# dylkot/cNMF

Hardware: AMD Instinct MI355X
Metric: NMF restarts/sec (50000x2000xK5..13) (higher is better)
Workload: dtype f32 (exact integer f16 plane x 2 f16 planes with per-row exponent, f32 accumulate)

## Files before the change

cnmf_amd/csrc/batch_host.hip.h:

```cpp
#pragma once

#include "batch_sched.h"

static_assert(PLAN_BK == BK && PLAN_G3_MW == G3_MW && PLAN_G3_JW == G3_JW && PLAN_G3C_JW == G3C_JW && PLAN_G3_BK == G3_BK &&
              PLAN_KSMALL == KSMALL, "pass_plan.h repeats the tile constants of the kernel headers");
static PadShape pad_shape(const cnmf_ctx* ctx) { return PadShape{ctx->N_pad, ctx->G_pad}; }
static int sweep_chunks(const cnmf_ctx* ctx, int L) { return sweep_chunks(ctx->knobs.sweep_parts, L); }
static int sweep_parts(const cnmf_ctx* ctx, int L) { return sweep_parts(ctx->knobs.sweep_parts, L); }

static int ensure_batch(cnmf_ctx* ctx, int KC, int max_k = KMAX, int min_k = 1)
{
    const bool use3 = gemm3_enabled(ctx, KC);
    const SplitCaps caps = size_splits(pad_shape(ctx), KC, use3, gemm3_wg_slots(ctx->knobs));
    const int nsplit = caps.nsplit, nsplitA = caps.nsplitA;
    const int parts = std::max(sweep_parts(ctx, (int)ctx->N), sweep_parts(ctx, (int)ctx->G));
    const size_t gp_need = (size_t)(KC / std::max(1, min_k) + 1) * parts * max_k * max_k;
    if (ctx->bat.kc == KC && ctx->bat.nsplit == nsplit && ctx->bat.nsplitA == nsplitA &&
        ctx->bat.parts == parts && ctx->bat.gram_part_floats >= gp_need && (!use3 || ctx->bat.H3)) return CNMF_OK;
    ctx->bat.release();
    OwnedLocal<BatchBuffersF> b;
    const size_t hb = (size_t)KC * ctx->G_pad * sizeof(float);
    const size_t wb = (size_t)KC * ctx->N_pad * sizeof(float);
    HIP_TRY(ctx, hipMalloc(&b.H, hb));
    HIP_TRY(ctx, hipMalloc(&b.Wt, wb));
// ... 62 lines not shown
        clk::time_point t0;
        bool timing = false;
        while (*flag != stamp) {
            if (++spins % 4096 != 0) continue;
            if (!timing) { t0 = clk::now(); timing = true; continue; }
            if (std::chrono::duration_cast<std::chrono::milliseconds>(clk::now() - t0).count() < 20) continue;
            t0 = clk::now();
            const hipError_t q = hipStreamQuery(ctx->stream);
            if (q == hipSuccess) {
                if (*flag == stamp) break;
                SET_ERR(ctx, "slot snapshot %d was never published (slot %d)", stamp, s);
                return CNMF_EHIP;
            }
            if (q != hipErrorNotReady) {
                SET_ERR(ctx, "stream failed while waiting for a slot snapshot: %s", hipGetErrorString(q));
                return CNMF_EHIP;
            }
        }
    }
    __atomic_thread_fence(__ATOMIC_ACQUIRE);
    return CNMF_OK;
}

static int validate_params(cnmf_ctx* ctx, const cnmf_cd_params* p)
{
    if (!p) { SET_ERR(ctx, "params is NULL"); return CNMF_EINVAL; }
    if (!(p->tol >= 0) || p->max_iter < 1) { SET_ERR(ctx, "bad tol/max_iter"); return CNMF_EINVAL; }
    if (p->l1_reg_W < 0 || p->l2_reg_W < 0 || p->l1_reg_H < 0 || p->l2_reg_H < 0) {
        SET_ERR(ctx, "negative regularisation"); return CNMF_EINVAL;
    }
    return CNMF_OK;
}

static_assert(SCHED_KMAX == KMAX && SCHED_RING == RING, "batch_sched.h repeats KMAX and RING");

struct PassScheme {
    bool use3 = false;
    bool usec = false;
    bool use2g = false;
    bool use2h = false;
    int mode = 0;
    XOperand xA{}, xB{};
    const double* dsc = nullptr;
    int jwA = G3_JW;
    int nsubA = 1, nsubB = 1, KbA = 0, KbB = 0;
    void leave_matrix_pipe() { use3 = usec = use2h = use2g = false; }
};

static int pick_scheme(cnmf_ctx* ctx, int KC, PassScheme* out)
{
    const CdKnobs& kn = ctx->knobs;
    PassScheme p;
    int rc;
    p.use3 = gemm3_enabled(ctx, KC);
    if (p.use3 && kn.gemm3 >= 3) {
        if ((rc = ensure_counts(ctx))) return rc;
        p.usec = ctx->counts.state == 1;
    }
    p.use2g = p.use3 && !p.usec && kn.gemm3 >= 4 && ctx->G_pad % G3C_JW == 0 && ctx->N_pad % G3C_JW == 0;
    if (p.use2g && (rc = ensure_x2planes(ctx))) return rc;
    p.use2h = (p.usec && ctx->counts.fmt == 4) || p.use2g;
    p.mode = !p.use3 ? 0 : (p.use2g ? 5 : (p.usec ? (p.use2h ? 4 : 3) : std::min(kn.gemm3, 2)));
    p.KbA = ctx->G_pad / 16; p.KbB = ctx->N_pad / 16;
    p.xA = p.use2g ? ctx->x2.passA() : ctx->counts.passA();
    p.xB = p.use2g ? ctx->x2.passB() : ctx->counts.passB();
    p.dsc = p.use2g ? nullptr : ctx->counts.d_scale;
    p.nsubA = p.use2h ? gemm2h_nsub(p.xA.hi != nullptr, p.KbA, kn.g2_nsub) : 1;
    p.nsubB = p.use2h ? gemm2h_nsub(p.xB.hi != nullptr, p.KbB, kn.g2_nsub) : 1;
    if (p.use3 && !p.usec && !p.use2g && (rc = ensure_planes(ctx))) return rc;
    p.jwA = (p.usec || p.use2g) ? G3C_JW : G3_JW;
    *out = p;
    return CNMF_OK;
}

struct BatchRun {
    cnmf_ctx* ctx; const cnmf_cd_params* prm; hipStream_t st;
    int n; const int32_t* kk; int init_mode; const double* avg; const float *W0, *H0;
    int32_t* n_iter_out; double* viol_out; bool resident;
    int N, G, max_k; int64_t total_k;
    std::vector<size_t> hoff, woff;
    DevPool pool;
    EventPool events;
    struct PinnedInts { int* p = nullptr; ~PinnedInts() { if (p) hipHostFree(p); } } repack_host;
    float *d_Hres = nullptr, *d_Wres = nullptr;
    float *d_H0 = nullptr, *d_Wt0 = nullptr;
    int* d_repack = nullptr;
    int n_repack = 0;
    PassScheme ps;
    bool fuseW = false;
    int shgen = 0;
    int* shW[2] = {nullptr, nullptr};
    bool h3_valid = false;
    int fin_y = 1, lag = 2;
    int chunksW, partsW, chunksH, partsH;
    float l1W, l2W, l1H, l2H;
    PassPlan plan;
    int time_stride = 0;
    std::vector<hipEvent_t> gev;
    hipEvent_t ev_begin = nullptr, ev_end = nullptr, ev_tail = nullptr;
    int nsplit3_first = 1;
    BatchSched sched;
    BatchRun(int n_, const int32_t* kk_, int KC, const double* hint, bool dbg) : n(n_), kk(kk_), sched(n_, kk_, KC, hint, dbg) {}
};

static int plan_passes(BatchRun& b, int cap, int capA)
{
    cnmf_ctx* ctx = b.ctx;
    PassPlan& p = b.plan;
    plan_pass_splits(p, pad_shape(ctx), b.sched.KC, b.ps.use3, b.ps.jwA, b.ps.nsubA, gemm3_wg_slots(ctx->knobs), ctx->knobs.no_streamk, cap, capA);
    const std::vector<unsigned char>* flags = b.ps.use3 ? (p.sk3.on ? &p.sk3.flags : nullptr) : (p.sk.on ? &p.sk.split : nullptr);
    if (flags) HIP_TRY(ctx, hipMemcpyAsync(ctx->bat.d_split, flags->data(), flags->size(), hipMemcpyHostToDevice, b.st));
    return CNMF_OK;
}

static int retire_slot(BatchRun& b, int s, const SlotDesc& snap)
{
    cnmf_ctx* ctx = b.ctx;
    hipStream_t st = b.st;
    const HostSlot& h = b.sched.hs[s];
    const int r = h.restart, k = h.k, N = b.N, G = b.G;
    dim3 gH((G + 255) / 256, k), gW((N + 255) / 256, k);
    extract_kernel<<<gH, 256, 0, st>>>(ctx->bat.H, ctx->G_pad, G, h.off, k, b.d_Hres + b.hoff[r], 0);
    if (b.d_Wres) extract_kernel<<<gW, 256, 0, st>>>(ctx->bat.Wt, ctx->N_pad, N, h.off, k, b.d_Wres + b.woff[r], 1);
    clear_rows_kernel<<<gH, 256, 0, st>>>(ctx->bat.H, ctx->G_pad, ctx->G_pad, h.off, k);
    clear_rows_kernel<<<gW, 256, 0, st>>>(ctx->bat.Wt, ctx->N_pad, ctx->N_pad, h.off, k);
    HIP_TRY(ctx, hipGetLastError());
    if (b.n_iter_out) b.n_iter_out[r] = snap.iter;
    if (b.viol_out) b.viol_out[r] = snap.viol_last;
    b.sched.retire(s, snap.iter);
    return CNMF_OK;
}

static int repack(BatchRun& b, int width, bool balanced = false)
{
    cnmf_ctx* ctx = b.ctx;
    hipStream_t st = b.st;
    const int KC0 = b.sched.KC0;
    int* hm = b.repack_host.p + (size_t)(b.n_repack++ % RING) * 3 * KC0;
    int* d_colmap = b.d_repack, *d_ids = b.d_repack + KC0, *d_offs = b.d_repack + 2 * KC0;
    const RepackPlan pl = b.sched.plan_repack(width, balanced, hm);
    if (pl.nmove || pl.pos < width) {
        HIP_TRY(ctx, hipMemcpyAsync(d_colmap, hm, (size_t)width * sizeof(int), hipMemcpyHostToDevice, st));
        gather_rows_cm_kernel<<<dim3((ctx->N_pad / 4 + 255) / 256, width), 256, 0, st>>>(ctx->bat.Wt, ctx->N_pad, d_colmap, ctx->bat.XHt);
        gather_rows_cm_kernel<<<dim3((ctx->G_pad / 4 + 255) / 256, width), 256, 0, st>>>(ctx->bat.H, ctx->G_pad, d_colmap, ctx->bat.XtW);
        HIP_TRY(ctx, hipGetLastError());
        HIP_TRY(ctx, hipMemcpyAsync(ctx->bat.Wt, ctx->bat.XHt, (size_t)width * ctx->N_pad * sizeof(float), hipMemcpyDeviceToDevice, st));
        HIP_TRY(ctx, hipMemcpyAsync(ctx->bat.H, ctx->bat.XtW, (size_t)width * ctx->G_pad * sizeof(float), hipMemcpyDeviceToDevice, st));
        if (b.fuseW) {
            int* tmp = ctx->bat.shiftW + 2 * ctx->bat.kc;
            for (int g2 = 0; g2 < 2; ++g2) {
                permute_ints_kernel<<<(width + 255) / 256, 256, 0, st>>>(b.shW[g2], d_colmap, tmp, width);
                HIP_TRY(ctx, hipMemcpyAsync(b.shW[g2], tmp, (size_t)width * sizeof(int), hipMemcpyDeviceToDevice, st));
            }
            HIP_TRY(ctx, hipGetLastError());
        }
        if (pl.nmove) {
            HIP_TRY(ctx, hipMemcpyAsync(d_ids, hm + KC0, (size_t)pl.nmove * sizeof(int), hipMemcpyHostToDevice, st));
            HIP_TRY(ctx, hipMemcpyAsync(d_offs, hm + 2 * KC0, (size_t)pl.nmove * sizeof(int), hipMemcpyHostToDevice, st));
            set_slot_offs_kernel<<<(pl.nmove + 255) / 256, 256, 0, st>>>(ctx->bat.d_slots, d_ids, d_offs, pl.nmove);
            HIP_TRY(ctx, hipGetLastError());
        }
    }
    b.h3_valid = false;
    if (b.ps.use2h) HIP_TRY(ctx, launch_rowmax_part(st, ctx->bat.Wt, ctx->N_pad, b.N, b.sched.KC, b.chunksW * 256, nullptr, b.partsW, ctx->bat.rmaxW));
    return CNMF_OK;
}

static int install(BatchRun& b, const Placement& p)
{
    cnmf_ctx* ctx = b.ctx;
    hipStream_t st = b.st;
    const int r = p.restart, k = p.k, off = p.off, N = b.N, G = b.G;
    dim3 gI((std::max(N, G) + 255) / 256, k);
    if (b.init_mode == 0) {
        HIP_TRY(ctx, hipMemcpyAsync(ctx->stageH, b.H0 + b.hoff[r], (size_t)k * G * sizeof(float), hipMemcpyHostToDevice, st));
        HIP_TRY(ctx, hipMemcpyAsync(ctx->stageW, b.W0 + b.woff[r], (size_t)k * N * sizeof(float), hipMemcpyHostToDevice, st));
        install_kernel<<<gI, 256, 0, st>>>(ctx->stageH, ctx->stageW, ctx->bat.H, ctx->G_pad, G, ctx->bat.Wt, ctx->N_pad, N, off, k);
    } else {
        install_cm_kernel<<<gI, 256, 0, st>>>(b.d_H0 + b.hoff[r], b.d_Wt0 + b.woff[r], ctx->bat.H, ctx->G_pad, G, ctx->bat.Wt, ctx->N_pad, N, off);
    }
    HIP_TRY(ctx, hipGetLastError());
    if (b.fuseW) {
        float mx = 0.f;
        if (b.init_mode == 1) mx = 6.0f * (float)b.avg[r];
        else for (size_t q = 0; q < (size_t)k * N; ++q) mx = std::max(mx, b.W0[b.woff[r] + q]);
        int e2 = 0;
        if (mx > 0.f) std::frexp(mx, &e2);
        const int sh0 = mx > 0.f ? std::max(-110, std::min(120, 13 - e2)) : 0;
        set_ints_kernel<<<1, 128, 0, st>>>(b.shW[0], b.shW[1], off, k, sh0);
        HIP_TRY(ctx, hipGetLastError());
    }
    SlotDesc* d = &ctx->bat.h_slots[p.slot];
    memset(d, 0, sizeof *d);
    d->off = off; d->k = k; d->active = 1; d->iter = 0; d->restart = r;
    HIP_TRY(ctx, hipMemcpyAsync(ctx->bat.d_slots + p.slot, d, sizeof(SlotDesc), hipMemcpyHostToDevice, st));
    return CNMF_OK;
}

static int refill(BatchRun& b, int& n_new)
{
    cnmf_ctx* ctx = b.ctx;
    BatchSched& sc = b.sched;
    n_new = 0;
    int* new_list = ctx->bat.h_slot_list + (size_t)(sc.it % RING) * sc.KC0;
    int rc;
    sc.begin_refill();
    while (true) {
        Placement p;
        while (sc.next_placement(&p)) {
            if ((rc = install(b, p))) return rc;
            new_list[n_new++] = p.slot;
        }
        if (!sc.defrag_due()) break;
        if ((rc = repack(b, sc.KC))) return rc;
        sc.defragmented();
    }
    if (n_new) {
        int* dl = ctx->bat.d_slot_list + (size_t)(sc.it % RING) * sc.KC0;
        HIP_TRY(ctx, hipMemcpyAsync(dl, new_list, n_new * sizeof(int), hipMemcpyHostToDevice, b.st));
        gram_rows_kernel<<<n_new, 256, 0, b.st>>>(ctx->bat.H, ctx->G_pad, b.G, ctx->bat.d_slots, dl, ctx->bat.gramH, b.l2W);
        HIP_TRY(ctx, hipGetLastError());
    }
    return CNMF_OK;
}

static int launch_pass_a(BatchRun& b, int n_new, unsigned long long livemask, hipEvent_t ev_begin, CutPlanes* cutA)
{
    cnmf_ctx* ctx = b.ctx;
    hipStream_t st = b.st;
    const PassScheme& ps = b.ps;
    const PassPlan& pl = b.plan;
    const int KC = b.sched.KC, gm = ctx->knobs.gemm3;
    const long long plane = (long long)KC * ctx->N_pad;
    *cutA = NO_CUT;
    if (!ps.use3) {
        if (pl.sk.on) {
            HIP_TRY(ctx, launch_streamk_passA(st, pl.sk, ctx->bat.H, ctx->G_pad, ctx->X, ctx->G_pad, ctx->bat.XHt,
                                              ctx->bat.XHt1, ctx->N_pad, ctx->N_pad));
            *cutA = CutPlanes{ctx->bat.XHt1, ctx->bat.d_split, 128, pl.sk.mw, pl.sk.MG, nullptr};
        } else
            HIP_TRY(ctx, launch_gemm<false>(st, 0, ctx->bat.H, ctx->G_pad, ctx->X, ctx->G_pad, ctx->bat.XHt,
                                            ctx->N_pad, plane, KC, ctx->G_pad, ctx->N_pad, pl.nsplitA));
        return CNMF_OK;
    }
    if ((n_new > 0 || !b.h3_valid) && ps.use2h) {
        HIP_TRY(ctx, launch_rowmax_part(st, ctx->bat.H, ctx->G_pad, b.G, KC, b.chunksH * 256, ps.dsc, b.partsH, ctx->bat.rmaxH));
        HIP_TRY(ctx, launch_split2h(st, ctx->bat.H, ctx->G_pad, KC, ctx->G_pad, ctx->bat.H3, G3_MW, ps.dsc, ctx->bat.rmaxH,
                                    b.partsH, ctx->bat.iscaleH));
    } else if (n_new > 0 || !b.h3_valid)
        HIP_TRY(ctx, launch_split3(st, ctx->bat.H, ctx->G_pad, KC, ctx->G_pad, ctx->bat.H3, G3_MW, ps.usec ? ctx->counts.d_scale : nullptr));
    if (ev_begin) hipEventRecord(ev_begin, st);
    if (ps.use2h) {
        G2Launch g;
        g.A2 = ctx->bat.H3; g.rscale = ctx->bat.iscaleH; g.x = ps.xA; g.Kb = ps.KbA;
        g.C[0] = ctx->bat.XHt; g.C[1] = ctx->bat.XHt1; g.C[2] = ctx->bat.XHt2; g.ldc = ctx->N_pad;
        g.livemask = livemask; g.kn = &ctx->knobs;
        if (pl.sk3.on) { g.sk = &pl.sk3; HIP_TRY(ctx, launch_gemm2h_streamk(st, g)); }
        else { g.cstride = plane; g.KC = KC; g.Jpad = ctx->N_pad; g.nsplit = pl.nsplitA; HIP_TRY(ctx, launch_gemm2h(st, g)); }
    } else if (pl.sk3.on) {
        if (ps.usec)
            HIP_TRY(ctx, launch_gemm3c_streamk(st, pl.sk3, ctx->bat.H3, ps.xA.plane, ps.xA.hi, ps.xA.flags, ctx->bat.XHt, ctx->bat.XHt1,
                                               ctx->bat.XHt2, ctx->N_pad));
        else
            HIP_TRY(ctx, launch_gemm3_streamk(st, pl.sk3, ctx->bat.H3, ctx->planes.X3, ctx->bat.XHt, ctx->bat.XHt1, ctx->bat.XHt2, ctx->N_pad, gm));
    } else if (ps.usec)
        HIP_TRY(ctx, launch_gemm3c(st, ctx->bat.H3, ps.xA.plane, ps.xA.hi, ps.xA.flags, ctx->G_pad / 16, ctx->bat.XHt, ctx->N_pad,
                                   plane, KC, ctx->N_pad, pl.nsplitA));
    else
        HIP_TRY(ctx, launch_gemm3(st, ctx->bat.H3, ctx->planes.X3, ctx->G_pad / 16, ctx->bat.XHt, ctx->N_pad,
                                  plane, KC, ctx->N_pad, pl.nsplitA, gm));
    if (pl.sk3.on) *cutA = CutPlanes{ctx->bat.XHt1, ctx->bat.d_split, ps.jwA, G3_MW, pl.sk3.MG, ctx->bat.XHt2};
    return CNMF_OK;
}

static void launch_finalize(BatchRun& b, const FinalizeArgs& fa)
{
    finalize_kernel<<<dim3(b.sched.nslots, b.fin_y), 256, 0, b.st>>>(fa.gram_part, fa.viol_part, fa.nparts, fa.gram_out, fa.l2_reg,
                                                                   fa.slots, fa.phase, fa.tol, fa.max_iter, fa.want_gram, fa.gld,
                                                                   fa.snap_out, fa.stamp);
}

static int launch_w_finalize(BatchRun& b)
{
    cnmf_ctx* ctx = b.ctx;
    const int KC = b.sched.KC, nslots = b.sched.nslots;
    const FinalizeArgs fa{ctx->bat.gram_part, ctx->bat.viol_part, b.partsW, ctx->bat.gramW, b.l2H, ctx->bat.d_slots, 0, b.prm->tol,
                          b.prm->max_iter, 1, b.max_k, nullptr, 0};
    if (b.ps.use2h) {
        const bool fuse_now = b.fuseW;
// ... 59 lines not shown
        HIP_TRY(ctx, launch_reduce_splits(b.st, ctx->bat.XtW, nsB, plane, plane, ps.usec ? ps.dsc : nullptr, ctx->G_pad));
    HIP_TRY(ctx, launch_sweep(b.st, s));
    return CNMF_OK;
}

static int launch_h_finalize(BatchRun& b)
{
    cnmf_ctx* ctx = b.ctx;
    const PassScheme& ps = b.ps;
    const BatchSched& sc = b.sched;
    SlotDesc* snap = ctx->bat.h_snap + (size_t)(sc.it % RING) * sc.KC0;
    SlotDesc* snap_dev = nullptr;
    HIP_TRY(ctx, hipHostGetDevicePointer((void**)&snap_dev, snap, 0));
    const FinalizeArgs fa{ctx->bat.gram_part, ctx->bat.viol_part, b.partsH, ctx->bat.gramH, b.l2W, ctx->bat.d_slots, 1, b.prm->tol,
                          b.prm->max_iter, 1, b.max_k, snap_dev, (int)(sc.it + 1)};
    if (ps.use2h)
        HIP_TRY(ctx, launch_split2h_finalize(b.st, ctx->bat.H, ctx->G_pad, sc.KC, ctx->G_pad, ctx->bat.H3, G3_MW, ps.dsc,
                                             ctx->bat.rmaxH, b.partsH, ctx->bat.iscaleH, fa, sc.nslots, b.fin_y));
    else if (ps.use3)
        HIP_TRY(ctx, launch_split3_finalize(b.st, ctx->bat.H, ctx->G_pad, sc.KC, ctx->G_pad, ctx->bat.H3, G3_MW,
                                            ps.usec ? ctx->counts.d_scale : nullptr, fa, sc.nslots, b.fin_y));
    else
        launch_finalize(b, fa);
    if (ps.use3) b.h3_valid = true;
    HIP_TRY(ctx, hipGetLastError());
    return CNMF_OK;
}

static int iterate(BatchRun& b, int n_new)
{
    cnmf_ctx* ctx = b.ctx;
    hipStream_t st = b.st;
    const PassScheme& ps = b.ps;
    BatchSched& sc = b.sched;
    int tiers = 0, rc;
    for (int s2 = 0; s2 < sc.nslots; ++s2)
        if (sc.hs[s2].state) tiers |= sc.hs[s2].k <= 16 ? 1 : (sc.hs[s2].k <= 32 ? 2 : (sc.hs[s2].k <= KSMALL ? 4 : 8));
    unsigned long long livemask = ~0ull;
    if (ps.use2h && sc.n_pending == 0 && ctx->knobs.part) {
        int fullest = 0;
        livemask = sc.live_tiles(&fullest);
        if (fullest > 6) livemask = ~0ull;
    }
    hipEvent_t* ev = nullptr;
    if (b.time_stride > 0 && sc.it % b.time_stride == 0) {
        for (int i = 0; i < 4; ++i) b.gev.push_back(b.events.get());
        POOL_TRY(ctx, b.events);
        ev = &b.gev[b.gev.size() - 4];
        hipEventRecord(ev[0], st);
    }
    SweepLaunch w = batch_sweep(ctx, sc.nslots, b.max_k, tiers);
    if ((rc = launch_pass_a(b, n_new, livemask, ev ? ev[0] : nullptr, &w.cut))) return rc;
    if (ev) hipEventRecord(ev[1], st);
    if (w.cut.plane1) w.from = SweepLaunch::CUT_PLANES;
    else
        HIP_TRY(ctx, launch_reduce_splits(st, ctx->bat.XHt, ps.use2h ? gemm2h_splits(ps.KbA, b.plan.nsplitA, ps.nsubA) : b.plan.nsplitA,
                                          (long long)sc.KC * ctx->N_pad, (long long)sc.KC * ctx->N_pad));
    w.V = ctx->bat.Wt; w.ldv = ctx->N_pad; w.L = b.N; w.P = ctx->bat.XHt; w.gram = ctx->bat.gramH; w.l1 = b.l1W;
    w.chunks = b.chunksW; w.parts = b.partsW; w.want_gram = 1;
    if (ps.use2h) w.rmax_part = ctx->bat.rmaxW;
    const PlaneOut wplanes{(unsigned short*)ctx->bat.Wt3, b.shW[b.shgen], ps.KbB, G3_MW};
    if (b.fuseW && ps.use2h) w.planes = &wplanes;
    HIP_TRY(ctx, launch_sweep(st, w));
    if ((rc = launch_w_finalize(b))) return rc;
    if (ev) hipEventRecord(ev[2], st);
    int nsB = 1;
    if ((rc = launch_pass_b(b, livemask, &nsB))) return rc;
    if (ev) hipEventRecord(ev[3], st);
    if ((rc = launch_h_sweep(b, tiers, nsB))) return rc;
    if ((rc = launch_h_finalize(b))) return rc;
    sc.end_iteration();
    return CNMF_OK;
}

static int inspect(BatchRun& b)
{
    BatchSched& sc = b.sched;
    const int64_t si = sc.it - 1 - b.lag;
    if (si < 0) return CNMF_OK;
    const SlotDesc* sp = b.ctx->bat.h_snap + (size_t)(si % RING) * sc.KC0;
    const int ns = sc.snap_nslots[si % RING];
    int rc = wait_snapshot(b.ctx, sp, ns, (int)(si + 1));
    if (rc) return rc;
    for (int s = 0; s < ns; ++s)
        if (sc.retirable(s, si, sp[s].active, sp[s].restart) && (rc = retire_slot(b, s, sp[s]))) return rc;
    sc.resort_pending();
    return CNMF_OK;
}

static int compact(BatchRun& b)
{
    BatchSched& sc = b.sched;
    PassScheme& ps = b.ps;
    if (!sc.in_tail()) return CNMF_OK;
    const bool part = b.ctx->knobs.part;
    const TailPlan t = sc.tail_plan(ps.use3, ps.usec, ps.use2h, part);
    int rc;
    if (t.rebalance) {
        if ((rc = repack(b, sc.KC, true))) return rc;
        sc.rebalanced();
    }
    if (t.width < sc.KC) {
        const int KC0 = sc.KC0;
        if ((rc = repack(b, t.width, t.stay3 && ps.use2h && part))) return rc;
        sc.narrowed(t.width);
        if (!t.stay3) ps.leave_matrix_pipe();
        if ((rc = plan_passes(b, (b.ctx->bat.nsplit * KC0) / sc.KC, (b.ctx->bat.nsplitA * KC0) / sc.KC))) return rc;
    }
    return CNMF_OK;
}

static int alloc_call_buffers(BatchRun& b, bool want_W)
{
    cnmf_ctx* ctx = b.ctx;
    const int G = b.G, n = b.n, KC0 = b.sched.KC0;
    if (b.resident) {
        if (ctx->spectra_rows && ctx->spectra_G != G) {
            SET_ERR(ctx, "the resident store holds spectra over %lld genes, this matrix has %d: cnmf_spectra_reset first",
                    (long long)ctx->spectra_G, G);
            return CNMF_ESTATE;
        }
        ctx->spectra_G = G;
        const size_t need = (ctx->spectra_rows + (size_t)b.total_k) * G;
        if (need > ctx->spectra_cap) {
            float* nb = nullptr;
            const size_t cap = std::max(need, ctx->spectra_cap * 2);
            HIP_TRY(ctx, hipMalloc(&nb, cap * sizeof(float)));
            hipError_t ce = hipSuccess;
            if (ctx->spectra_rows)
                ce = hipMemcpyAsync(nb, ctx->spectra, ctx->spectra_rows * G * sizeof(float), hipMemcpyDeviceToDevice, b.st);
            if (ce == hipSuccess) ce = hipStreamSynchronize(b.st);
            if (ce != hipSuccess) { hipFree(nb); HIP_TRY(ctx, ce); }
            hipFree(ctx->spectra);
            ctx->spectra = nb; ctx->spectra_cap = cap;
        }
        b.d_Hres = ctx->spectra + ctx->spectra_rows * G;
    } else {
        b.d_Hres = b.pool.get<float>(b.hoff[n]);
    }
    if (want_W) b.d_Wres = b.pool.get<float>(b.woff[n]);
    b.d_repack = b.pool.get<int>((size_t)3 * KC0);
    POOL_TRY(ctx, b.pool);
    HIP_TRY(ctx, hipHostMalloc(&b.repack_host.p, (size_t)RING * 3 * KC0 * sizeof(int)));
    return CNMF_OK;
}

static int generate_inits(BatchRun& b, const uint32_t* seeds)
{
    cnmf_ctx* ctx = b.ctx;
    const int n = b.n, N = b.N, G = b.G;
    b.d_H0 = b.pool.get<float>(b.hoff[n]);
    b.d_Wt0 = b.pool.get<float>(b.woff[n]);
    RngJob* d_jobs = b.pool.get<RngJob>((size_t)n);
    POOL_TRY(ctx, b.pool);
    std::vector<RngJob> jobs(n);
    int rowoff = 0;
    for (int r = 0; r < n; ++r) {
        jobs[r] = RngJob{seeds[r], b.kk[r], rowoff, b.avg[r], (long long)b.kk[r] * ((long long)G + N)};
        rowoff += b.kk[r];
    }
    HIP_TRY(ctx, hipMemcpy(d_jobs, jobs.data(), (size_t)n * sizeof(RngJob), hipMemcpyHostToDevice));
    rng_kernel<1><<<n, 256, 0, b.st>>>(d_jobs, nullptr, b.d_H0, G, G, b.d_Wt0, N, N);
    HIP_TRY(ctx, hipGetLastError());
    return CNMF_OK;
}

static int pick_batch_width(cnmf_ctx* ctx, const cnmf_cd_params* prm, int64_t total_k, int max_k, int* KC_out)
{
    const CdKnobs& kn = ctx->knobs;
    const bool wide_can = kn.gemm3 != 0 && gemm3_enabled(ctx, 512);
    const bool wide_small = total_k >= 512 && kn.wide_small;
    const bool wide_auto = wide_can && ((int64_t)ctx->N_pad * ctx->G_pad >= (1ll << 24) || wide_small);
    int KC = pick_kc(kn.kc, kn.kc_limit, total_k, max_k, prm->kc_max, (prm->kc_max > 256 || kn.kc_set) ? wide_can : wide_auto);
    if (KC == 128 && prm->kc_max <= 0 && !kn.kc_set && kn.gemm3 >= 3 && gemm3_enabled(ctx, 256) &&
        (int64_t)ctx->N_pad * ctx->G_pad >= (1ll << 24)) {
        int rc = ensure_counts(ctx);
        if (rc) return rc;
        if (ctx->counts.state == 1) KC = 256;
    }
    *KC_out = KC;
    return CNMF_OK;
}

static int finish_batch(BatchRun& b, float* H_out, float* W_out, cnmf_batch_stats* stats)
{
    cnmf_ctx* ctx = b.ctx;
    const BatchSched& sc = b.sched;
    if (sc.dbg) sc.print_debug();
    HIP_TRY(ctx, hipEventRecord(b.ev_end, b.st));
    if (!b.resident)
        HIP_TRY(ctx, hipMemcpyAsync(H_out, b.d_Hres, b.hoff[b.n] * sizeof(float), hipMemcpyDeviceToHost, b.st));
    if (W_out)
        HIP_TRY(ctx, hipMemcpyAsync(W_out, b.d_Wres, b.woff[b.n] * sizeof(float), hipMemcpyDeviceToHost, b.st));
    HIP_TRY(ctx, hipStreamSynchronize(b.st));
    if (b.resident) ctx->spectra_rows += (size_t)b.total_k;
    if (ctx->iter_prior.size() != (size_t)KMAX + 1) ctx->iter_prior.assign((size_t)KMAX + 1, 0.0);
    for (int k = 1; k <= KMAX; ++k)
        if (sc.k_done[k]) ctx->iter_prior[k] = (double)sc.k_iters[k] / (double)sc.k_done[k];
    if (!stats) return CNMF_OK;
    float ms = 0.f;
    hipEventElapsedTime(&ms, b.ev_begin, b.ev_end);
    stats->gpu_ms = ms;
    stats->outer_iterations = sc.it;
    stats->restart_iterations = sc.restart_iters;
    stats->column_iterations = sc.column_iters;
    stats->restart_column_iterations = sc.restart_col_iters;
    stats->kc = sc.KC0; stats->nsplit = b.ps.mode ? b.nsplit3_first : ctx->bat.nsplit;
    stats->gemm_mode = b.ps.mode;
    stats->tail_iterations = sc.tail_its; stats->tail_live_columns = sc.tail_live;
    if (b.ev_tail) { float tms = 0.f; hipEventElapsedTime(&tms, b.ev_tail, b.ev_end); stats->tail_ms = tms; }
    for (size_t i = 0; i + 3 < b.gev.size(); i += 4) {
        float a = 0.f, c = 0.f;
        hipEventElapsedTime(&a, b.gev[i], b.gev[i + 1]);
        hipEventElapsedTime(&c, b.gev[i + 2], b.gev[i + 3]);
        stats->passA_ms += a; stats->passB_ms += c;
        stats->passA_launches++; stats->passB_launches++;
    }
    return CNMF_OK;
}

static int run_batch(cnmf_ctx* ctx, int n, const int32_t* kk, int init_mode, const uint32_t* seeds,
                     const double* avg, const float* W0, const float* H0, const cnmf_cd_params* prm,
                     float* H_out, float* W_out, bool resident, int32_t* n_iter_out,
                     double* viol_out, cnmf_batch_stats* stats)
{
    if (!ctx) { SET_ERR(ctx, "ctx is NULL"); return CNMF_EINVAL; }
    if (int rcd_ = ensure_dense(ctx)) return rcd_;
    const CdKnobs& kn = ctx->knobs;
    int rc = validate_params(ctx, prm);
    if (rc) return rc;
    if (n < 0 || (n > 0 && !kk)) { SET_ERR(ctx, "bad restart list"); return CNMF_EINVAL; }
    if (init_mode == 0 && n > 0 && (!W0 || !H0)) { SET_ERR(ctx, "init_mode 0 needs W0 and H0"); return CNMF_EINVAL; }
    if (init_mode == 1 && n > 0 && (!seeds || !avg)) { SET_ERR(ctx, "init_mode 1 needs seeds and avg"); return CNMF_EINVAL; }
    if (init_mode != 0 && init_mode != 1) { SET_ERR(ctx, "unknown init_mode %d", init_mode); return CNMF_EINVAL; }
    if (!resident && n > 0 && !H_out) { SET_ERR(ctx, "H_out is NULL"); return CNMF_EINVAL; }
    HIP_TRY(ctx, hipSetDevice(ctx->device));
    if (stats) memset(stats, 0, sizeof *stats);
    if (n == 0) return CNMF_OK;

    const int N = (int)ctx->N, G = (int)ctx->G;
    int64_t total_k = 0; int max_k = 0, min_k = 1 << 30;
    std::vector<size_t> hoff(n + 1, 0), woff(n + 1, 0);
    for (int r = 0; r < n; ++r) {
        if (kk[r] < 1) { SET_ERR(ctx, "n_components must be >= 1 (restart %d)", r); return CNMF_EINVAL; }
        if (kk[r] > KMAX) { SET_ERR(ctx, "n_components=%d > CNMF_KMAX=%d is not supported by the device sweep", kk[r], KMAX); return CNMF_EUNSUPPORTED; }
// ... 158 lines not shown
```

cnmf_amd/csrc/kernels_sweep.hip.h:

```cpp
#pragma once
#include <hip/hip_runtime.h>
#include "kernels_gemm.hip.h"
#include "kernels_gemm2h.hip.h"

namespace cnmf {

constexpr int KMAX = 128;
constexpr int KSMALL = 64;
constexpr int GRAM_LD = KMAX;
constexpr int GRAM_SZ = KMAX * KMAX;

static inline int sweep_kg(int kmax) { return kmax <= 16 ? 16 : (kmax <= 32 ? 32 : 64); }
static inline int sweep_wstride(int kmax) { return sweep_kg(kmax) + 1; }
static inline size_t sweep_lds_bytes(int kmax, bool planes = false)
{
    const int kg = sweep_kg(kmax);
    if (planes)
        return sweep_lds_bytes(kmax, false) + sizeof(float) * (size_t)(4 * kg * 64 + kg);
    return sizeof(float) * (size_t)(kg * (kg + 4) + 8 + 256 + 4 * (kg == 16 ? 32 : 64) * sweep_wstride(kmax));
}

struct SlotDesc {
    int off;
    int k;
// ... 651 lines not shown
    }
    if (by != 0) return;
    double v = 0.0;
    for (int pI = tid; pI < nparts; pI += 256) v += viol_part[(size_t)slot * nparts + pI];
    red[tid] = v;
    __syncthreads();
    for (int o = 128; o > 0; o >>= 1) {
        if (tid < o) red[tid] += red[tid + o];
        __syncthreads();
    }
    if (tid == 0) {
        const double vsum = red[0];
        if (phase == 0) {
            sd->viol = vsum;
        } else {
            const double viol = (phase == 1) ? sd->viol + vsum : vsum;
            const int it = sd->iter + 1;
            sd->iter = it;
            if (it == 1) sd->viol_init = viol;
            bool done = false;
            if (sd->viol_init == 0.0) { done = true; sd->viol_last = 0.0; }
            else {
                sd->viol_last = viol / sd->viol_init;
                if (sd->viol_last <= tol) done = true;
            }
            if (it >= max_iter) done = true;
            sd->viol = 0.0;
            if (done) sd->active = 0;
        }
        if (snap_out) publish_slot(snap_out + slot, *sd, stamp);
    }
}

__global__ __launch_bounds__(256) void finalize_kernel(
    const float* __restrict__ gram_part, const double* __restrict__ viol_part, int nparts,
    float* __restrict__ gram_out, float l2_reg,
    SlotDesc* __restrict__ slots, int phase, double tol, int max_iter, int want_gram, int gld,
    SlotDesc* snap_out = nullptr, int stamp = 0)
{
    __shared__ double red[256];
    const FinalizeArgs a{gram_part, viol_part, nparts, gram_out, l2_reg, slots, phase, tol, max_iter, want_gram, gld,
                         snap_out, stamp};
    finalize_body(a, blockIdx.x, blockIdx.y, red);
}

__global__ __launch_bounds__(256) void split3_finalize_kernel(const float* __restrict__ src, int ld, int K, int TR,
                                                              unsigned short* __restrict__ dst,
                                                              const double* __restrict__ kscale, int split_bx,
                                                              int split_by, FinalizeArgs fa, int fin_y)
{
    __shared__ __attribute__((aligned(16))) unsigned char lds[4 * 64 * 48 * 2];
    const int b = blockIdx.x, nsplit = split_bx * split_by;
    if (b < nsplit) {
        split3_tiled_body(src, ld, K, TR, dst, kscale, b % split_bx, b / split_bx,
                          reinterpret_cast<unsigned short (*)[64][48]>(lds));
    } else {
        const int f = b - nsplit;
        finalize_body(fa, f / fin_y, f % fin_y, reinterpret_cast<double*>(lds));
    }
}

template <int TROWS, int TKB>
__global__ __launch_bounds__(256) void split2h_finalize_kernel(const float* __restrict__ src, int ld, int K, int TR,
                                                               unsigned short* __restrict__ dst,
                                                               const double* __restrict__ kscale,
                                                               const float* __restrict__ rmax_part, int parts,
                                                               float* __restrict__ inv_scale, int split_bx,
                                                               int split_by, FinalizeArgs fa, int fin_y,
                                                               SplitFused fu = SplitFused{nullptr, nullptr})
{
    __shared__ __attribute__((aligned(16))) unsigned char lds[256 * 32 * 2];
    const int b = blockIdx.x, nsplit = split_bx * split_by;
    if (b < nsplit) {
        split2h_tiled_body<TROWS, TKB>(src, ld, K, TR, dst, kscale, rmax_part, parts, inv_scale, b % split_bx, split_bx,
                                       b / split_bx, reinterpret_cast<unsigned short*>(lds),
                                       reinterpret_cast<float*>(lds), fu);
    } else {
        const int f = b - nsplit;
        finalize_body(fa, f / fin_y, f % fin_y, reinterpret_cast<double*>(lds));
    }
}

template <int KR, int GC>
__device__ __forceinline__ void gram_rows_body(const float* __restrict__ V, int ldv, int L, int k, int off, int slot,
                                               float* __restrict__ gram_out, float l2_reg, float* lds)
{
    float (*tile)[GC + 1] = reinterpret_cast<float (*)[GC + 1]>(lds);
    const int tid = threadIdx.x;
    constexpr int NP = KR * KR / 256;
    double acc[NP];
#pragma unroll
    for (int i = 0; i < NP; ++i) acc[i] = 0.0;
    for (int g0 = 0; g0 < L; g0 += GC) {
        for (int e = tid; e < k * GC; e += 256) {
            const int c = e / GC, g = e % GC;
            tile[c][g] = (g0 + g < L) ? V[(size_t)(off + c) * ldv + g0 + g] : 0.f;
        }
        __syncthreads();
#pragma unroll
        for (int i = 0; i < NP; ++i) {
            const int e = tid + 256 * i;
            if (e < k * k) {
                const int a = e / k, b = e % k;
                float s = 0.f;
                for (int g = 0; g < GC; ++g) s = fmaf(tile[a][g], tile[b][g], s);
                acc[i] += (double)s;
            }
        }
        __syncthreads();
    }
#pragma unroll
    for (int i = 0; i < NP; ++i) {
        const int e = tid + 256 * i;
        if (e < k * k) {
            const int a = e / k, b = e % k;
            float s = (float)acc[i];
            if (a == b) s += l2_reg;
            gram_out[(size_t)slot * GRAM_SZ + a * GRAM_LD + b] = s;
        }
    }
}

__global__ __launch_bounds__(256) void gram_rows_kernel(
    const float* __restrict__ V, int ldv, int L,
    const SlotDesc* __restrict__ slots, const int* __restrict__ slot_list,
    float* __restrict__ gram_out, float l2_reg)
{
    const int slot = slot_list[blockIdx.x];
    const SlotDesc sd = slots[slot];
    __shared__ __attribute__((aligned(16))) float lds[KSMALL * 129];
    if (sd.k <= KSMALL) gram_rows_body<KSMALL, 128>(V, ldv, L, sd.k, sd.off, slot, gram_out, l2_reg, lds);
    else gram_rows_body<KMAX, 64>(V, ldv, L, sd.k, sd.off, slot, gram_out, l2_reg, lds);
}

__global__ void install_kernel(const float* __restrict__ H0, const float* __restrict__ W0,
                               float* __restrict__ H, int ldh, int G,
                               float* __restrict__ Wt, int ldw, int N, int off, int k)
{
    const int c = blockIdx.y;
    const int i = blockIdx.x * blockDim.x + threadIdx.x;
    if (i < G) H[(size_t)(off + c) * ldh + i] = H0 ? H0[(size_t)c * G + i] : 0.f;
    if (i < N) Wt[(size_t)(off + c) * ldw + i] = W0 ? W0[(size_t)i * k + c] : 0.f;
}

__global__ void install_cm_kernel(const float* __restrict__ H0, const float* __restrict__ Wt0,
                                  float* __restrict__ H, int ldh, int G,
                                  float* __restrict__ Wt, int ldw, int N, int off)
{
    const int c = blockIdx.y;
    const int i = blockIdx.x * blockDim.x + threadIdx.x;
    if (i < G) H[(size_t)(off + c) * ldh + i] = H0[(size_t)c * G + i];
    if (i < N) Wt[(size_t)(off + c) * ldw + i] = Wt0[(size_t)c * N + i];
}

__global__ void set_slot_off_kernel(SlotDesc* slots, int slot, int off) { slots[slot].off = off; }

__global__ __launch_bounds__(256) void gather_rows_cm_kernel(const float* __restrict__ V, int ld,
                                                             const int* __restrict__ colmap, float* __restrict__ stage)
{
    const int j = blockIdx.y, i = (blockIdx.x * 256 + threadIdx.x) * 4;
    if (i >= ld) return;
    const int c = colmap[j];
    float4 v = make_float4(0.f, 0.f, 0.f, 0.f);
    if (c >= 0) v = *reinterpret_cast<const float4*>(V + (size_t)c * ld + i);
    *reinterpret_cast<float4*>(stage + (size_t)j * ld + i) = v;
}

__global__ void set_ints_kernel(int* __restrict__ a, int* __restrict__ b, int off, int n, int value)
{
    const int i = blockIdx.x * blockDim.x + threadIdx.x;
    if (i < n) { a[off + i] = value; b[off + i] = value; }
}
__global__ void permute_ints_kernel(const int* __restrict__ src, const int* __restrict__ colmap, int* __restrict__ dst, int n)
{
    const int j = blockIdx.x * blockDim.x + threadIdx.x;
    if (j < n) { const int c = colmap[j]; dst[j] = c >= 0 ? src[c] : 0; }
}

__global__ void set_slot_offs_kernel(SlotDesc* slots, const int* __restrict__ ids, const int* __restrict__ offs, int n)
{
    const int i = blockIdx.x * blockDim.x + threadIdx.x;
    if (i < n) slots[ids[i]].off = offs[i];
}

__global__ void clear_rows_kernel(float* __restrict__ V, int ldv, int L, int off, int k)
{
    const int c = blockIdx.y;
    const int i = blockIdx.x * blockDim.x + threadIdx.x;
    if (c < k && i < L) V[(size_t)(off + c) * ldv + i] = 0.f;
}

__global__ void extract_kernel(const float* __restrict__ V, int ldv, int L, int off, int k,
                               float* __restrict__ out, int transpose)
{
    const int c = blockIdx.y;
    const int i = blockIdx.x * blockDim.x + threadIdx.x;
    if (c < k && i < L) {
        const float v = V[(size_t)(off + c) * ldv + i];
        if (transpose) out[(size_t)i * k + c] = v; else out[(size_t)c * L + i] = v;
    }
}

__global__ void pad_copy_kernel(const float* __restrict__ src, int rows, int cols,
                                float* __restrict__ dst, int ld)
{
    const int r = blockIdx.y;
    const int c = blockIdx.x * blockDim.x + threadIdx.x;
    if (r < rows && c < cols) dst[(size_t)r * ld + c] = src[(size_t)r * cols + c];
}

}
```

Before: 224.9.

## Batch slot install and retire into single launches, precompute start Grams, swap W buffers

Per-restart install and retire launches are replaced by job tables copied once per refill or retire event and handled by one batched kernel each. Rows map to jobs through a binary search. For on-device init, the starting H Gram matrices are computed up front by a new kernel, and the install kernel writes the Gram, W exponents and slot descriptor directly, which removes many small launches and host syncs. In repack, when nsplitA==1 the W staging buffer is swapped with the live one instead of copied, which adds a gather over all KC0 rows and relies on both buffers having the same size.

Measured after the change: 227.1, median of 6. About the same (+1.0%).

```diff
diff --git a/cnmf_amd/csrc/batch_host.hip.h b/cnmf_amd/csrc/batch_host.hip.h
--- a/cnmf_amd/csrc/batch_host.hip.h
+++ b/cnmf_amd/csrc/batch_host.hip.h
@@ -168,8 +168,12 @@
     DevPool pool;
     EventPool events;
     struct PinnedInts { int* p = nullptr; ~PinnedInts() { if (p) hipHostFree(p); } } repack_host;
+    InstallJob *h_install = nullptr, *d_install = nullptr;
+    RetireJob *h_retire = nullptr, *d_retire = nullptr;
     float *d_Hres = nullptr, *d_Wres = nullptr;
     float *d_H0 = nullptr, *d_Wt0 = nullptr;
+    float* d_gram0 = nullptr;
+    std::vector<long long> goff;
     int* d_repack = nullptr;
     int n_repack = 0;
     PassScheme ps;
@@ -199,21 +203,24 @@
     return CNMF_OK;
 }
 
-static int retire_slot(BatchRun& b, int s, const SlotDesc& snap)
-{
-    cnmf_ctx* ctx = b.ctx;
-    hipStream_t st = b.st;
+static void retire_slot(BatchRun& b, int s, const SlotDesc& snap, RetireJob* jobs, int* njobs, int* rows)
+{
     const HostSlot& h = b.sched.hs[s];
-    const int r = h.restart, k = h.k, N = b.N, G = b.G;
-    dim3 gH((G + 255) / 256, k), gW((N + 255) / 256, k);
-    extract_kernel<<<gH, 256, 0, st>>>(ctx->bat.H, ctx->G_pad, G, h.off, k, b.d_Hres + b.hoff[r], 0);
-    if (b.d_Wres) extract_kernel<<<gW, 256, 0, st>>>(ctx->bat.Wt, ctx->N_pad, N, h.off, k, b.d_Wres + b.woff[r], 1);
-    clear_rows_kernel<<<gH, 256, 0, st>>>(ctx->bat.H, ctx->G_pad, ctx->G_pad, h.off, k);
-    clear_rows_kernel<<<gW, 256, 0, st>>>(ctx->bat.Wt, ctx->N_pad, ctx->N_pad, h.off, k);
-    HIP_TRY(ctx, hipGetLastError());
+    const int r = h.restart;
+    jobs[(*njobs)++] = RetireJob{h.off, h.k, *rows, 0, (long long)b.hoff[r], (long long)b.woff[r]};
+    *rows += h.k;
     if (b.n_iter_out) b.n_iter_out[r] = snap.iter;
     if (b.viol_out) b.viol_out[r] = snap.viol_last;
     b.sched.retire(s, snap.iter);
+}
+
+static int launch_retire(BatchRun& b, const RetireJob* jobs, int njobs, int rows)
+{
+    cnmf_ctx* ctx = b.ctx;
+    HIP_TRY(ctx, hipMemcpyAsync(b.d_retire, jobs, (size_t)njobs * sizeof(RetireJob), hipMemcpyHostToDevice, b.st));
+    retire_event_kernel<<<dim3((std::max(ctx->N_pad, ctx->G_pad) + 255) / 256, rows), 256, 0, b.st>>>(
+        b.d_retire, njobs, ctx->bat.H, ctx->G_pad, b.G, ctx->bat.Wt, ctx->N_pad, b.N, b.d_Hres, b.d_Wres);
+    HIP_TRY(ctx, hipGetLastError());
     return CNMF_OK;
 }
 
@@ -226,11 +233,15 @@
     int* d_colmap = b.d_repack, *d_ids = b.d_repack + KC0, *d_offs = b.d_repack + 2 * KC0;
     const RepackPlan pl = b.sched.plan_repack(width, balanced, hm);
     if (pl.nmove || pl.pos < width) {
-        HIP_TRY(ctx, hipMemcpyAsync(d_colmap, hm, (size_t)width * sizeof(int), hipMemcpyHostToDevice, st));
-        gather_rows_cm_kernel<<<dim3((ctx->N_pad / 4 + 255) / 256, width), 256, 0, st>>>(ctx->bat.Wt, ctx->N_pad, d_colmap, ctx->bat.XHt);
+        const bool swapW = ctx->bat.nsplitA == 1;
+        const int wrows = swapW ? KC0 : width;
+        for (int c = width; c < wrows; ++c) hm[c] = -1;
+        HIP_TRY(ctx, hipMemcpyAsync(d_colmap, hm, (size_t)wrows * sizeof(int), hipMemcpyHostToDevice, st));
+        gather_rows_cm_kernel<<<dim3((ctx->N_pad / 4 + 255) / 256, wrows), 256, 0, st>>>(ctx->bat.Wt, ctx->N_pad, d_colmap, ctx->bat.XHt);
         gather_rows_cm_kernel<<<dim3((ctx->G_pad / 4 + 255) / 256, width), 256, 0, st>>>(ctx->bat.H, ctx->G_pad, d_colmap, ctx->bat.XtW);
         HIP_TRY(ctx, hipGetLastError());
-        HIP_TRY(ctx, hipMemcpyAsync(ctx->bat.Wt, ctx->bat.XHt, (size_t)width * ctx->N_pad * sizeof(float), hipMemcpyDeviceToDevice, st));
+        if (swapW) std::swap(ctx->bat.Wt, ctx->bat.XHt);
+        else HIP_TRY(ctx, hipMemcpyAsync(ctx->bat.Wt, ctx->bat.XHt, (size_t)width * ctx->N_pad * sizeof(float), hipMemcpyDeviceToDevice, st));
         HIP_TRY(ctx, hipMemcpyAsync(ctx->bat.H, ctx->bat.XtW, (size_t)width * ctx->G_pad * sizeof(float), hipMemcpyDeviceToDevice, st));
         if (b.fuseW) {
             int* tmp = ctx->bat.shiftW + 2 * ctx->bat.kc;
@@ -252,28 +263,28 @@
     return CNMF_OK;
 }
 
+static int first_w_exponent(const BatchRun& b, int r, int k)
+{
+    float mx = 0.f;
+    if (b.init_mode == 1) mx = 6.0f * (float)b.avg[r];
+    else for (size_t q = 0; q < (size_t)k * b.N; ++q) mx = std::max(mx, b.W0[b.woff[r] + q]);
+    int e2 = 0;
+    if (mx > 0.f) std::frexp(mx, &e2);
+    return mx > 0.f ? std::max(-110, std::min(120, 13 - e2)) : 0;
+}
+
 static int install(BatchRun& b, const Placement& p)
 {
     cnmf_ctx* ctx = b.ctx;
     hipStream_t st = b.st;
     const int r = p.restart, k = p.k, off = p.off, N = b.N, G = b.G;
     dim3 gI((std::max(N, G) + 255) / 256, k);
-    if (b.init_mode == 0) {
-        HIP_TRY(ctx, hipMemcpyAsync(ctx->stageH, b.H0 + b.hoff[r], (size_t)k * G * sizeof(float), hipMemcpyHostToDevice, st));
-        HIP_TRY(ctx, hipMemcpyAsync(ctx->stageW, b.W0 + b.woff[r], (size_t)k * N * sizeof(float), hipMemcpyHostToDevice, st));
-        install_kernel<<<gI, 256, 0, st>>>(ctx->stageH, ctx->stageW, ctx->bat.H, ctx->G_pad, G, ctx->bat.Wt, ctx->N_pad, N, off, k);
-    } else {
-        install_cm_kernel<<<gI, 256, 0, st>>>(b.d_H0 + b.hoff[r], b.d_Wt0 + b.woff[r], ctx->bat.H, ctx->G_pad, G, ctx->bat.Wt, ctx->N_pad, N, off);
-    }
+    HIP_TRY(ctx, hipMemcpyAsync(ctx->stageH, b.H0 + b.hoff[r], (size_t)k * G * sizeof(float), hipMemcpyHostToDevice, st));
+    HIP_TRY(ctx, hipMemcpyAsync(ctx->stageW, b.W0 + b.woff[r], (size_t)k * N * sizeof(float), hipMemcpyHostToDevice, st));
+    install_kernel<<<gI, 256, 0, st>>>(ctx->stageH, ctx->stageW, ctx->bat.H, ctx->G_pad, G, ctx->bat.Wt, ctx->N_pad, N, off, k);
     HIP_TRY(ctx, hipGetLastError());
     if (b.fuseW) {
-        float mx = 0.f;
-        if (b.init_mode == 1) mx = 6.0f * (float)b.avg[r];
-        else for (size_t q = 0; q < (size_t)k * N; ++q) mx = std::max(mx, b.W0[b.woff[r] + q]);
-        int e2 = 0;
-        if (mx > 0.f) std::frexp(mx, &e2);
-        const int sh0 = mx > 0.f ? std::max(-110, std::min(120, 13 - e2)) : 0;
-        set_ints_kernel<<<1, 128, 0, st>>>(b.shW[0], b.shW[1], off, k, sh0);
+        set_ints_kernel<<<1, 128, 0, st>>>(b.shW[0], b.shW[1], off, k, first_w_exponent(b, r, k));
         HIP_TRY(ctx, hipGetLastError());
     }
     SlotDesc* d = &ctx->bat.h_slots[p.slot];
@@ -283,14 +294,44 @@
     return CNMF_OK;
 }
 
+static int launch_install(BatchRun& b, const InstallJob* jobs, int njobs, int rows)
+{
+    cnmf_ctx* ctx = b.ctx;
+    HIP_TRY(ctx, hipMemcpyAsync(b.d_install, jobs, (size_t)njobs * sizeof(InstallJob), hipMemcpyHostToDevice, b.st));
+    install_event_kernel<<<dim3((std::max(b.N, b.G) + 255) / 256, rows), 256, 0, b.st>>>(
+        b.d_install, njobs, b.d_H0, b.d_Wt0, b.d_gram0, ctx->bat.H, ctx->G_pad, b.G, ctx->bat.Wt, ctx->N_pad, b.N,
+        b.fuseW ? b.shW[0] : nullptr, b.fuseW ? b.shW[1] : nullptr, ctx->bat.d_slots, ctx->bat.gramH);
+    HIP_TRY(ctx, hipGetLastError());
+    return CNMF_OK;
+}
+
 static int refill(BatchRun& b, int& n_new)
 {
     cnmf_ctx* ctx = b.ctx;
     BatchSched& sc = b.sched;
     n_new = 0;
-    int* new_list = ctx->bat.h_slot_list + (size_t)(sc.it % RING) * sc.KC0;
     int rc;
     sc.begin_refill();
+    if (b.init_mode == 1) {
+        InstallJob* jobs = b.h_install + (size_t)(sc.it % RING) * sc.KC0;
+        int first = 0, rows = 0;
+        while (true) {
+            Placement p;
+            while (sc.next_placement(&p)) {
+                const int r = p.restart;
+                jobs[n_new++] = InstallJob{p.slot, r, p.off, p.k, (long long)b.hoff[r], (long long)b.woff[r], b.goff[r],
+                                           b.fuseW ? first_w_exponent(b, r, p.k) : 0, rows};
+                rows += p.k;
+            }
+            if (n_new > first && (rc = launch_install(b, jobs + first, n_new - first, rows))) return rc;
+            first = n_new; rows = 0;
+            if (!sc.defrag_due()) break;
+            if ((rc = repack(b, sc.KC))) return rc;
+            sc.defragmented();
+        }
+        return CNMF_OK;
+    }
+    int* new_list = ctx->bat.h_slot_list + (size_t)(sc.it % RING) * sc.KC0;
     while (true) {
         Placement p;
         while (sc.next_placement(&p)) {
@@ -516,8 +557,11 @@
     const int ns = sc.snap_nslots[si % RING];
     int rc = wait_snapshot(b.ctx, sp, ns, (int)(si + 1));
     if (rc) return rc;
+    RetireJob* jobs = b.h_retire + (size_t)(sc.it % RING) * sc.KC0;
+    int njobs = 0, rows = 0;
     for (int s = 0; s < ns; ++s)
-        if (sc.retirable(s, si, sp[s].active, sp[s].restart) && (rc = retire_slot(b, s, sp[s]))) return rc;
+        if (sc.retirable(s, si, sp[s].active, sp[s].restart)) retire_slot(b, s, sp[s], jobs, &njobs, &rows);
+    if (njobs && (rc = launch_retire(b, jobs, njobs, rows))) return rc;
     sc.resort_pending();
     return CNMF_OK;
 }
@@ -574,8 +618,13 @@
     }
     if (want_W) b.d_Wres = b.pool.get<float>(b.woff[n]);
     b.d_repack = b.pool.get<int>((size_t)3 * KC0);
+    b.d_install = b.pool.get<InstallJob>((size_t)KC0);
+    b.d_retire = b.pool.get<RetireJob>((size_t)KC0);
     POOL_TRY(ctx, b.pool);
-    HIP_TRY(ctx, hipHostMalloc(&b.repack_host.p, (size_t)RING * 3 * KC0 * sizeof(int)));
+    const size_t ints = (size_t)RING * 3 * KC0 * sizeof(int), inst = (size_t)RING * KC0 * sizeof(InstallJob);
+    HIP_TRY(ctx, hipHostMalloc(&b.repack_host.p, ints + inst + (size_t)RING * KC0 * sizeof(RetireJob)));
+    b.h_install = reinterpret_cast<InstallJob*>(reinterpret_cast<char*>(b.repack_host.p) + ints);
+    b.h_retire = reinterpret_cast<RetireJob*>(reinterpret_cast<char*>(b.repack_host.p) + ints + inst);
     return CNMF_OK;
 }
 
@@ -586,15 +635,23 @@
     b.d_H0 = b.pool.get<float>(b.hoff[n]);
     b.d_Wt0 = b.pool.get<float>(b.woff[n]);
     RngJob* d_jobs = b.pool.get<RngJob>((size_t)n);
-    POOL_TRY(ctx, b.pool);
+    StartGramJob* d_gjobs = b.pool.get<StartGramJob>((size_t)n);
     std::vector<RngJob> jobs(n);
+    std::vector<StartGramJob> gjobs(n);
+    b.goff.assign((size_t)n + 1, 0);
     int rowoff = 0;
     for (int r = 0; r < n; ++r) {
         jobs[r] = RngJob{seeds[r], b.kk[r], rowoff, b.avg[r], (long long)b.kk[r] * ((long long)G + N)};
+        gjobs[r] = StartGramJob{(long long)b.hoff[r], b.goff[r], b.kk[r], 0};
+        b.goff[r + 1] = b.goff[r] + (long long)b.kk[r] * b.kk[r];
         rowoff += b.kk[r];
     }
+    b.d_gram0 = b.pool.get<float>((size_t)b.goff[n]);
+    POOL_TRY(ctx, b.pool);
     HIP_TRY(ctx, hipMemcpy(d_jobs, jobs.data(), (size_t)n * sizeof(RngJob), hipMemcpyHostToDevice));
+    HIP_TRY(ctx, hipMemcpy(d_gjobs, gjobs.data(), (size_t)n * sizeof(StartGramJob), hipMemcpyHostToDevice));
     rng_kernel<1><<<n, 256, 0, b.st>>>(d_jobs, nullptr, b.d_H0, G, G, b.d_Wt0, N, N);
+    start_gram_kernel<<<n, 256, 0, b.st>>>(b.d_H0, G, d_gjobs, b.d_gram0, b.l2W);
     HIP_TRY(ctx, hipGetLastError());
     return CNMF_OK;
 }
diff --git a/cnmf_amd/csrc/kernels_sweep.hip.h b/cnmf_amd/csrc/kernels_sweep.hip.h
--- a/cnmf_amd/csrc/kernels_sweep.hip.h
+++ b/cnmf_amd/csrc/kernels_sweep.hip.h
@@ -757,8 +757,8 @@
 }
 
 template <int KR, int GC>
-__device__ __forceinline__ void gram_rows_body(const float* __restrict__ V, int ldv, int L, int k, int off, int slot,
-                                               float* __restrict__ gram_out, float l2_reg, float* lds)
+__device__ __forceinline__ void gram_rows_body(const float* __restrict__ V, int ldv, int L, int k, int off,
+                                               float* __restrict__ gram_out, int gld, float l2_reg, float* lds)
 {
     float (*tile)[GC + 1] = reinterpret_cast<float (*)[GC + 1]>(lds);
     const int tid = threadIdx.x;
@@ -791,7 +791,7 @@
             const int a = e / k, b = e % k;
             float s = (float)acc[i];
             if (a == b) s += l2_reg;
-            gram_out[(size_t)slot * GRAM_SZ + a * GRAM_LD + b] = s;
+            gram_out[a * gld + b] = s;
         }
     }
 }
@@ -804,8 +804,20 @@
     const int slot = slot_list[blockIdx.x];
     const SlotDesc sd = slots[slot];
     __shared__ __attribute__((aligned(16))) float lds[KSMALL * 129];
-    if (sd.k <= KSMALL) gram_rows_body<KSMALL, 128>(V, ldv, L, sd.k, sd.off, slot, gram_out, l2_reg, lds);
-    else gram_rows_body<KMAX, 64>(V, ldv, L, sd.k, sd.off, slot, gram_out, l2_reg, lds);
+    float* out = gram_out + (size_t)slot * GRAM_SZ;
+    if (sd.k <= KSMALL) gram_rows_body<KSMALL, 128>(V, ldv, L, sd.k, sd.off, out, GRAM_LD, l2_reg, lds);
+    else gram_rows_body<KMAX, 64>(V, ldv, L, sd.k, sd.off, out, GRAM_LD, l2_reg, lds);
+}
+
+struct StartGramJob { long long src, dst; int k, pad_; };
+
+__global__ __launch_bounds__(256) void start_gram_kernel(const float* __restrict__ H0, int G, const StartGramJob* __restrict__ jobs,
+                                                         float* __restrict__ store, float l2_reg)
+{
+    const StartGramJob j = jobs[blockIdx.x];
+    __shared__ __attribute__((aligned(16))) float lds[KSMALL * 129];
+    if (j.k <= KSMALL) gram_rows_body<KSMALL, 128>(H0 + j.src, G, G, j.k, 0, store + j.dst, j.k, l2_reg, lds);
+    else gram_rows_body<KMAX, 64>(H0 + j.src, G, G, j.k, 0, store + j.dst, j.k, l2_reg, lds);
 }
 
 __global__ void install_kernel(const float* __restrict__ H0, const float* __restrict__ W0,
@@ -818,17 +830,78 @@
     if (i < N) Wt[(size_t)(off + c) * ldw + i] = W0 ? W0[(size_t)i * k + c] : 0.f;
 }
 
-__global__ void install_cm_kernel(const float* __restrict__ H0, const float* __restrict__ Wt0,
-                                  float* __restrict__ H, int ldh, int G,
-                                  float* __restrict__ Wt, int ldw, int N, int off)
-{
-    const int c = blockIdx.y;
-    const int i = blockIdx.x * blockDim.x + threadIdx.x;
-    if (i < G) H[(size_t)(off + c) * ldh + i] = H0[(size_t)c * G + i];
-    if (i < N) Wt[(size_t)(off + c) * ldw + i] = Wt0[(size_t)c * N + i];
-}
-
 __global__ void set_slot_off_kernel(SlotDesc* slots, int slot, int off) { slots[slot].off = off; }
+
+struct InstallJob {
+    int slot, restart, off, k;
+    long long hoff, woff, goff;
+    int sh0, row0;
+};
+struct RetireJob {
+    int off, k, row0, pad_;
+    long long hdst, wdst;
+};
+
+template <typename J>
+__device__ __forceinline__ int job_of_row(const J* __restrict__ jobs, int n, int y)
+{
+    int lo = 0, hi = n - 1;
+    while (lo < hi) {
+        const int mid = (lo + hi + 1) >> 1;
+        if (jobs[mid].row0 <= y) lo = mid; else hi = mid - 1;
+    }
+    return lo;
+}
+
+__global__ __launch_bounds__(256) void install_event_kernel(const InstallJob* __restrict__ jobs, int njobs,
+                                                            const float* __restrict__ H0, const float* __restrict__ Wt0,
+                                                            const float* __restrict__ gram0,
+                                                            float* __restrict__ H, int ldh, int G,
+                                                            float* __restrict__ Wt, int ldw, int N,
+                                                            int* __restrict__ shA, int* __restrict__ shB,
+                                                            SlotDesc* __restrict__ slots, float* __restrict__ gramH)
+{
+    const int y = blockIdx.y;
+    const InstallJob j = jobs[job_of_row(jobs, njobs, y)];
+    const int c = y - j.row0;
+    if (c < 0 || c >= j.k) return;
+    const int i = blockIdx.x * 256 + threadIdx.x;
+    if (i < G) H[(size_t)(j.off + c) * ldh + i] = H0[j.hoff + (long long)c * G + i];
+    if (i < N) Wt[(size_t)(j.off + c) * ldw + i] = Wt0[j.woff + (long long)c * N + i];
+    if (blockIdx.x != 0) return;
+    if ((int)threadIdx.x < j.k)
+        gramH[(size_t)j.slot * GRAM_SZ + c * GRAM_LD + threadIdx.x] = gram0[j.goff + c * j.k + threadIdx.x];
+    if (threadIdx.x != 0) return;
+    if (shA) { shA[j.off + c] = j.sh0; shB[j.off + c] = j.sh0; }
+    if (c == 0) {
+        SlotDesc d;
+        d.off = j.off; d.k = j.k; d.active = 1; d.iter = 0; d.restart = j.restart; d.pad_ = 0;
+        d.viol = 0.0; d.viol_init = 0.0; d.viol_last = 0.0;
+        slots[j.slot] = d;
+    }
+}
+
+__global__ __launch_bounds__(256) void retire_event_kernel(const RetireJob* __restrict__ jobs, int njobs,
+                                                           float* __restrict__ H, int ldh, int G,
+                                                           float* __restrict__ Wt, int ldw, int N,
+                                                           float* __restrict__ Hres, float* __restrict__ Wres)
+{
+    const int y = blockIdx.y;
+    const RetireJob j = jobs[job_of_row(jobs, njobs, y)];
+    const int c = y - j.row0;
+    if (c < 0 || c >= j.k) return;
+    const int i = blockIdx.x * 256 + threadIdx.x;
+    if (i < ldh) {
+        float* p = H + (size_t)(j.off + c) * ldh + i;
+        if (i < G) Hres[j.hdst + (long long)c * G + i] = *p;
+        *p = 0.f;
+    }
+    if (i < ldw) {
+        float* p = Wt + (size_t)(j.off + c) * ldw + i;
+        if (Wres && i < N) Wres[j.wdst + (long long)i * j.k + c] = *p;
+        *p = 0.f;
+    }
+}
 
 __global__ __launch_bounds__(256) void gather_rows_cm_kernel(const float* __restrict__ V, int ld,
                                                              const int* __restrict__ colmap, float* __restrict__ stage)
```
